# ShreenathKR2000/DFU-Multimodal

Measured on AMD Instinct MI355X. Metric: images/sec (fusion fwd+bwd, bs=64/GPU), higher is better.
Workload: dtype fwd ResNet50 bf16x3, ViT-B/16 Blocks fp16 (fp32 accumulate, residual stream, statistics); bwd bf16 MFMA; fp32 master weights / AdamW

## Files before the change

### dfu-multimodal_amd/csrc/bn.hip

```cpp
#include "common.h"

namespace {

constexpr int FIN_WAVES = 16;

DFU_DEV void st_sc1_f64(double* p, double v) {
  __hip_atomic_store((unsigned long long*)p, (unsigned long long)__double_as_longlong(v),
                     __ATOMIC_RELAXED, __HIP_MEMORY_SCOPE_AGENT);
}
DFU_DEV double ld_sc1_f64(const double* p) {
  return __longlong_as_double((long long)__hip_atomic_load((unsigned long long*)p, __ATOMIC_RELAXED,
                                                          __HIP_MEMORY_SCOPE_AGENT));
}

DFU_DEV bool last_slice(int* counter, int S, int* flag) {
  asm volatile("s_waitcnt vmcnt(0)" ::: "memory");
  __syncthreads();
  if (threadIdx.x == 0) {
    const int old = __hip_atomic_fetch_add(counter, 1, __ATOMIC_RELAXED, __HIP_MEMORY_SCOPE_AGENT);
    const int last = old == S - 1;
    if (last) __hip_atomic_store(counter, 0, __ATOMIC_RELAXED, __HIP_MEMORY_SCOPE_AGENT);
    *flag = last;
  }
  __syncthreads();
// ... 295 lines not shown
    }
  };
  if (FIXED) load_coef((threadIdx.x & (cv - 1)) * 8);
  for (int64_t i = blockIdx.x * (int64_t)blockDim.x + threadIdx.x; i < n;
       i += (int64_t)gridDim.x * blockDim.x) {
    if (!FIXED) load_coef((int)(i % cv) * 8);
    float g[8], yy[8], oo[8];
    const u32x4 gv = *(const u32x4*)(dout + i * 8), yv = *(const u32x4*)(y + i * 8);
    u32x4 ov = {};
    if constexpr (RELU == 1) ov = *(const u32x4*)(out + i * 8);
    if constexpr (RELU == 3) ov[0] = ((const uint8_t*)out)[i];
    unpack8(gv, g);
    unpack8(yv, yy);
    unpack8(ov, oo);
    relu_mask8<RELU>(oo, yy, sc, sf, g, ov[0]);
    if (dres) *(u32x4*)(dres + i * 8) = pack8(g);
    float d[8];
#pragma unroll
    for (int e = 0; e < 8; ++e) d[e] = fmaf(ka[e], g[e], fmaf(kb[e], yy[e], kc[e]));
    *(u32x4*)(dy + i * 8) = pack8(d);
  }
}

__global__ __launch_bounds__(256) void k_bn_tile_stats(const bf16_t* __restrict__ x, int M, int C,
                                                       float* __restrict__ stats) {
  __shared__ float red[4][64];
  const int lane = threadIdx.x & 63, g = threadIdx.x >> 6;
  const int c = blockIdx.y * 64 + lane;
  const int r0 = blockIdx.x * 128, nb = min(128, M - r0);
  const int ra = r0 + g * 32, rb = min(r0 + nb, ra + 32);
  float v[32];
#pragma unroll
  for (int i = 0; i < 32; ++i) {
    const int r = ra + i;
    v[i] = (c < C && r < rb) ? bf2f(x[(int64_t)r * C + c]) : 0.f;
  }
  float s = 0.f;
#pragma unroll
  for (int i = 0; i < 32; ++i) s += v[i];
  red[g][lane] = s;
  __syncthreads();
  const float tot = red[0][lane] + red[1][lane] + red[2][lane] + red[3][lane];
  const float mu = tot / (float)nb;
  __syncthreads();
  float q = 0.f;
#pragma unroll
// ... 169 lines not shown
                          stream);
}

extern "C" int dfu_bn_bwd_apply(const void* dout, const void* y, const void* out, int32_t relu,
                                const float* scale, const float* shift, const float* mean,
                                const float* invstd, const float* coef, int64_t M, int32_t C,
                                void* dy, void* dres, void* stream) {
  DFU_CHECK_ARG(dout && y && mean && invstd && coef && dy && C % 8 == 0 && M > 0 && relu >= 0 &&
                    relu <= 3,
                "dfu_bn_bwd_apply: bad args");
  DFU_CHECK_ARG((relu != 1 && relu != 3) || out, "dfu_bn_bwd_apply: relu=1/3 needs out/mask");
  DFU_CHECK_ARG(relu != 2 || (scale && shift), "dfu_bn_bwd_apply: relu=2 needs scale/shift");
  const bool fx = fixed_channels(C);
  auto kern = relu == 1   ? (fx ? k_bn_bwd_apply<1, true> : k_bn_bwd_apply<1, false>)
              : relu == 2 ? (fx ? k_bn_bwd_apply<2, true> : k_bn_bwd_apply<2, false>)
              : relu == 3 ? (fx ? k_bn_bwd_apply<3, true> : k_bn_bwd_apply<3, false>)
                          : (fx ? k_bn_bwd_apply<0, true> : k_bn_bwd_apply<0, false>);
  hipLaunchKernelGGL(kern, dim3(grid_for(M * C / 8)), dim3(256), 0, (hipStream_t)stream,
                     (const bf16_t*)dout, (const bf16_t*)y, (const bf16_t*)out, scale, shift, mean,
                     invstd, coef, M, C, (bf16_t*)dy, (bf16_t*)dres);
  DFU_LAUNCH_CHECK();
  return DFU_OK;
}
```

### dfu-multimodal_amd/csrc/precise.hip

```cpp
#include "common.h"

namespace {

constexpr int TPB = 256;

inline unsigned nblocks(int64_t n, int per_block = TPB) {
  int64_t b = (n + per_block - 1) / per_block;
  if (b > 65535 * 4) b = 65535 * 4;
  return (unsigned)(b < 1 ? 1 : b);
}

DFU_DEV void split8(const float* f, float* hi, float* lo) {
#pragma unroll
  for (int e = 0; e < 8; ++e) {
    hi[e] = bf2f(f2bf(f[e]));
    lo[e] = f[e] - hi[e];
  }
}

DFU_DEV void st_triple8(bf16_t* row, int C, int c, const float* f, int pattern) {
  float hi[8], lo[8];
  split8(f, hi, lo);
  const u32x4 h = pack8(hi), l = pack8(lo);
  *(u32x4*)(row + c) = h;
// ... 67 lines not shown
    } else {
      bf16_t* o = out + t * 3 * C + c;
      o[0] = h;
      o[C] = h;
      o[2 * C] = l;
    }
  }
}

DFU_DEV void st_pair8(bf16_t* hi, bf16_t* lo, int64_t e, const float* f) {
  float h[8], l[8];
  split8(f, h, l);
  *(u32x4*)(hi + e) = pack8(h);
  *(u32x4*)(lo + e) = pack8(l);
}
DFU_DEV void ld8_pair(const bf16_t* hi, const bf16_t* lo, int64_t e, float* f) {
  float h[8], l[8];
  unpack8(*(const u32x4*)(hi + e), h);
  unpack8(*(const u32x4*)(lo + e), l);
#pragma unroll
  for (int i = 0; i < 8; ++i) f[i] = h[i] + l[i];
}

__global__ void k_bn_apply_x3(const void* __restrict__ y, const bf16_t* __restrict__ y_lo,
                              const float* __restrict__ scale,
                              const float* __restrict__ shift, const void* __restrict__ res,
                              const bf16_t* __restrict__ res_lo, int res_mode, int relu,
                              bf16_t* __restrict__ out_lo, bf16_t* __restrict__ out_bf,
                              float* __restrict__ out_f32, bf16_t* __restrict__ y_bf,
                              uint8_t* __restrict__ relu_mask, int64_t M, int C, int cv_log2) {
  const int cv = C / 8;
  const int64_t n = M * cv;
  for (int64_t i = blockIdx.x * (int64_t)blockDim.x + threadIdx.x; i < n;
       i += (int64_t)gridDim.x * blockDim.x) {
    const int64_t m = i >> cv_log2;
    const int c = (int)(i & (cv - 1)) * 8;
    const int64_t e = m * C + c;
    float f[8], r[8], sc[8], sh[8];
    {
      const f32x4 s0 = *(const f32x4*)(scale + c), s1 = *(const f32x4*)(scale + c + 4);
      const f32x4 h0 = *(const f32x4*)(shift + c), h1 = *(const f32x4*)(shift + c + 4);
#pragma unroll
      for (int k = 0; k < 4; ++k) {
        sc[k] = s0[k];
        sc[k + 4] = s1[k];
        sh[k] = h0[k];
        sh[k + 4] = h1[k];
      }
    }
    if (y_lo) {
      ld8_pair((const bf16_t*)y, y_lo, e, f);
    } else {
      ld8_f32((const float*)y + e, f);
      if (y_bf) *(u32x4*)(y_bf + e) = pack8(f);
    }
    if (res_mode == 1) ld8_f32((const float*)res + e, r);
    else if (res_mode == 2) ld8_pair((const bf16_t*)res, res_lo, e, r);
#pragma unroll
    for (int k = 0; k < 8; ++k) {
      float v = fmaf(f[k], sc[k], sh[k]);
      if (res_mode) v += r[k];
      f[k] = relu ? fmaxf(v, 0.f) : v;
    }
    if (out_lo) st_pair8(out_bf, out_lo, e, f);
    else if (out_bf) *(u32x4*)(out_bf + e) = pack8(f);
    if (out_f32) st8_f32(out_f32 + e, f);
    if (relu_mask) {
      unsigned bits = 0;
#pragma unroll
      for (int k = 0; k < 8; ++k) bits |= (unsigned)(f[k] > 0.f) << k;
      relu_mask[i] = (uint8_t)bits;
    }
  }
}

__global__ void k_maxpool_fwd_x3(const float* __restrict__ x, int B, int H, int W, int C,
                                 bf16_t* __restrict__ y_lo, bf16_t* __restrict__ y_bf,
                                 uint8_t* __restrict__ am, int P, int Q) {
  const int cv = C / 8;
  const int64_t n = (int64_t)B * P * Q * cv;
// ... 203 lines not shown
                    (pattern != 2 || seg % 32 == 0) &&
                    (!hi_out || (ld_hi % 8 == 0 && ld_hi >= seg)),
                "dfu_split_x3: bad args (seg %% 8 == 0, seg >= cols, pattern 0/1/2; 2: seg %% 32 == 0)");
  const int64_t n = (int64_t)rows * (seg / 8);
  if (n == 0) return DFU_OK;
  hipLaunchKernelGGL(k_split_x3, dim3(nblocks(n)), dim3(TPB), 0, (hipStream_t)stream, in, ld_in,
                     rows, cols, seg, (bf16_t*)out, pattern, (bf16_t*)hi_out, ld_hi);
  DFU_LAUNCH_CHECK();
  return DFU_OK;
}

extern "C" int dfu_pack_conv_weight_x3(const float* w, void* out, int32_t K, int32_t C, int32_t R,
                                       int32_t S, int32_t pattern, void* stream) {
  DFU_CHECK_ARG(w && out && K > 0 && C > 0 && R > 0 && S > 0 &&
                    (pattern == 1 || (pattern == 2 && C % 32 == 0)),
                "dfu_pack_conv_weight_x3: bad args (pattern 1, or 2 with C %% 32 == 0)");
  const int64_t n = (int64_t)K * R * S * C;
  hipLaunchKernelGGL(k_pack_conv_weight_x3, dim3(nblocks(n)), dim3(TPB), 0, (hipStream_t)stream,
                     w, (bf16_t*)out, K, C, R, S, pattern);
  DFU_LAUNCH_CHECK();
  return DFU_OK;
}

extern "C" int dfu_bn_apply_x3(const void* y, const void* y_lo, const float* scale,
                               const float* shift, const void* residual,
                               const void* residual_lo, int32_t res_mode,
                               int32_t relu, void* out_lo, void* out_bf16, float* out_f32,
                               void* y_bf16, uint8_t* relu_mask, int64_t M, int32_t C,
                               void* stream) {
  const int cv = C / 8;
  int cv_log2 = 0;
  while ((1 << cv_log2) < cv) ++cv_log2;
  DFU_CHECK_ARG(C % 8 == 0 && cv > 0 && (1 << cv_log2) == cv,
                "dfu_bn_apply_x3: C / 8 must be a power of two (C=%d)", C);
  DFU_CHECK_ARG((((uintptr_t)scale | (uintptr_t)shift) & 15) == 0,
                "dfu_bn_apply_x3: scale/shift must be 16-byte aligned");
  DFU_CHECK_ARG(y && scale && shift && C % 8 == 0 && M >= 0 && res_mode >= 0 && res_mode <= 2 &&
                    (res_mode == 0 || residual) && (res_mode != 2 || residual_lo) &&
                    (!out_lo || out_bf16),
                "dfu_bn_apply_x3: bad args");
  const int64_t n = M * (C / 8);
  if (n == 0) return DFU_OK;
  hipLaunchKernelGGL(k_bn_apply_x3, dim3(nblocks(n)), dim3(TPB), 0, (hipStream_t)stream, y,
                     (const bf16_t*)y_lo, scale, shift, residual, (const bf16_t*)residual_lo,
                     res_mode, relu, (bf16_t*)out_lo,
                     (bf16_t*)out_bf16, out_f32, (bf16_t*)y_bf16, relu_mask, M, C, cv_log2);
  DFU_LAUNCH_CHECK();
  return DFU_OK;
}

extern "C" int dfu_maxpool_fwd_x3(const float* x, int32_t B, int32_t H, int32_t W, int32_t C,
                                  void* y_lo, void* y_bf16, uint8_t* argmax, int32_t P, int32_t Q,
                                  void* stream) {
  DFU_CHECK_ARG(x && y_lo && y_bf16 && argmax && C % 8 == 0, "dfu_maxpool_fwd_x3: bad args");
  DFU_CHECK_ARG(P == (H - 1) / 2 + 1 && Q == (W - 1) / 2 + 1, "dfu_maxpool_fwd_x3: bad P/Q");
  const int64_t n = (int64_t)B * P * Q * (C / 8);
  hipLaunchKernelGGL(k_maxpool_fwd_x3, dim3(nblocks(n)), dim3(TPB), 0, (hipStream_t)stream, x, B,
                     H, W, C, (bf16_t*)y_lo, (bf16_t*)y_bf16, argmax, P, Q);
  DFU_LAUNCH_CHECK();
  return DFU_OK;
}

extern "C" int dfu_maxpool_bn_fwd_x3(const void* y, const void* y_lo, const float* scale,
                                     const float* shift, int32_t B, int32_t H, int32_t W,
                                     int32_t C, void* out_lo, void* out_bf16, uint8_t* argmax,
                                     uint8_t* relu_mask, int32_t P, int32_t Q, void* stream) {
  const int cv = C / 8;
  int cv_log2 = 0;
  while ((1 << cv_log2) < cv) ++cv_log2;
  DFU_CHECK_ARG(y && y_lo && scale && shift && out_lo && out_bf16 && argmax && C % 8 == 0 &&
                    cv > 0 && (1 << cv_log2) == cv && P == (H - 1) / 2 + 1 &&
// ... 65 lines not shown
```

### dfu-multimodal_amd/dfu_hip/functional.py

```python
import math
import os
import weakref

import torch

from . import _lib as L
from . import ops
from .streams import (current_stream, join_grad_streams, new_stream, on_stream,
                      side_stream, stream_wait, wgrad_stream)
from .grads import (arm_backward_join, disarm_backward_join, grad_buffer,
                    grad_or_none, grads_done, register_backward_end_hook,
                    register_grad_ready_hook, remove_backward_end_hook, remove_grad_ready_hook,
                    wants)
from .optim import x3_pair_weight

BF16 = torch.bfloat16
F32 = torch.float32

PRECISIONS = ("bf16", "bf16x3", "mixed", "parity")
STAGE_MODES = ("bf16", "bf16x3", "fp16")
DEFAULT_PRECISION = "parity"
_precision = [DEFAULT_PRECISION]


# ... 208 lines not shown
                w._dfu_shadow_x3_version = w._version
            return sh
    if _X3_PAIRS:
        if w.shape[2] == 1 and w.shape[3] == 1:
            return ops.split_x3(w.detach().reshape(w.shape[0], -1), ops.X3_PAIRS)
        return ops.pack_conv_weight_x3(w.detach(), ops.X3_PAIRS)
    if w.shape[2] == 1 and w.shape[3] == 1:
        return weight_x3_rows(w)
    return ops.pack_conv_weight_x3(w.detach())


def _take_x3(x):
    hi = rows_view(nhwc_bf16(x.detach()))
    lo = getattr(x, "_dfu_lo", None)
    if lo is not None:
        try:
            del x._dfu_lo
        except AttributeError:
            pass
        return hi, lo
    return hi, torch.zeros_like(hi)


class BNState:

    def __init__(self, bn, M, C, device):
        self.bn = bn
        self.M, self.C = M, C
        self.training = bn.training or not bn.track_running_stats
        self.coef4 = _empty((4, C), F32, device)
        self.scale, self.shift, self.mean, self.invstd = self.coef4.unbind(0)

    def forward_coeffs(self, stats):
        bn = self.bn
        if self.training:
            track = bn.track_running_stats and bn.training
            mom = bn.momentum if bn.momentum is not None else 0.1
            mp = module_param
            ops.bn_finalize(stats, self.M, self.C, mp(bn, "weight"), mp(bn, "bias"), bn.eps, mom,
                            mp(bn, "running_mean") if track else None,
                            mp(bn, "running_var") if track else None,
                            mp(bn, "num_batches_tracked") if track else None,
                            self.mean, self.invstd, self.scale, self.shift)
        else:
            ops.bn_eval_coeffs(bn.weight, bn.bias, bn.running_mean, bn.running_var, bn.eps,
                               self.scale, self.shift)
            self.mean.copy_(bn.running_mean)
            ops.bn_eval_coeffs(None, None, bn.running_mean, bn.running_var, bn.eps,
                               self.invstd, _empty((self.C,), F32, self.mean.device))

    def backward(self, dout, y, out, relu, dy, dres):
        bn = self.bn
        w, b = module_param(bn, "weight"), module_param(bn, "bias")
        dgamma = grad_or_none(w)
        dbeta = grad_or_none(b)
        ops.bn_bwd(dout, y, out, relu, self.mean, self.invstd, w, self.M, self.C, dy,
                   dres, dgamma, dbeta, batch_stats=self.training, scale=self.scale,
                   shift=self.shift)
        grads_done(w, b)


def gemm_wgrad(N, K, rows, dy, x, dw, ld_dy=None, ld_x=None):
    ops.gemm(N, K, rows, dy, N if ld_dy is None else ld_dy, x,
             x.stride(0) if ld_x is None else ld_x, dw, K, a_mode=L.OPND_MNMAJOR,
             b_mode=L.OPND_MNMAJOR, epilogue=L.EPI_F32_ACC)


def gemm_dgrad_f32(rows, N, K, dy, w):
    dx = _empty((rows, N), F32, dy.device)
    ops.gemm(rows, N, K, dy, K, w, N, dx, N, b_mode=L.OPND_MNMAJOR, epilogue=L.EPI_F32)
    return dx


def conv_fwd(x_rows, geom, w_krsc, y, stats):
    g = geom
    M = g.n * g.p * g.q
    if g.plain:
        ops.gemm(M, g.k, g.c, x_rows, g.c, w_krsc, g.c, y, g.k, epilogue=L.EPI_BF16_STATS,
                 stats=stats)
    else:
        K = g.r * g.s * g.c
        ops.gemm(M, g.k, K, x_rows, 0, w_krsc, K, y, g.k, a_mode=L.OPND_CONV_FWD,
# ... 171 lines not shown
        dx = im2col_conv_dx(dy, wb, g) if ctx.x_requires_grad else None
        return dx, None, None, None, None


def _fire_grad_hooks(probe, grad):
    for hook in list((probe._backward_hooks or {}).values()):
        hook(grad)


def conv_bn(xrows, geom, w, bnmod, relu, residual=None, mask=None):
    dev = xrows.device
    M = geom.n * geom.p * geom.q
    y = _empty((M, geom.k), BF16, dev)
    stats = _empty((ops.stats_tiles(M), 2, geom.k), F32, dev)
    conv_fwd(xrows, geom, w, y, stats)
    st = BNState(bnmod, M, geom.k, dev)
    st.forward_coeffs(stats)
    out = _empty((M, geom.k), BF16, dev)
    ops.bn_apply(y, st.scale, st.shift, residual, relu, out, M, geom.k, mask=mask)
    return y, out, st


def conv_bn_x3(xpair, geom, w3x, bnmod, relu, res=None, res_mode=0, want_pair=True,
               want_f32=False):
    dev = xpair[0].device
    M = geom.n * geom.p * geom.q
    y = _empty((M, geom.k), BF16, dev)
    y_lo = _empty((M, geom.k), BF16, dev)
    stats = _empty((ops.stats_tiles(M), 2, geom.k), F32, dev)
    conv_fwd_x3(xpair, geom, w3x, y, stats, y_lo=y_lo)
    st = BNState(bnmod, M, geom.k, dev)
    st.forward_coeffs(stats)
    out = _empty((M, geom.k), BF16, dev) if want_pair else None
    lo = _empty((M, geom.k), BF16, dev) if want_pair else None
    of = _empty((M, geom.k), F32, dev) if want_f32 else None
    rhi, rlo = res if res_mode == 2 else (res, None)
    mask = _empty((M * geom.k // 8,), torch.uint8, dev) if relu else None
    ops.bn_apply_x3(y, st.scale, st.shift, rhi, res_mode, relu, M, geom.k, out_lo=lo,
                    out_bf16=out, out_f32=of, residual_lo=rlo, y_lo=y_lo, relu_mask=mask)
    return y, out, lo, of, st, mask


class BottleneckFn(torch.autograd.Function):

    @staticmethod
    def forward(ctx, x, *params_and_mod):
        mod = params_and_mod[-1]
        mm = mod._modules
        x3mode = _x3(mod)
        xin3 = _take_x3(x) if x3mode else None
        x = nhwc_bf16(x.detach())
        B, Cin, H, W = x.shape
        xr = rows_view(x)
        g1 = _geom(mm["conv1"], B, H, W)
        g2 = _geom(mm["conv2"], B, g1.p, g1.q)
        g3 = _geom(mm["conv3"], B, g2.p, g2.q)
        down = mm.get("downsample")
        geo = (g1, g2, g3, _geom(down[0], B, H, W) if down is not None else None)
        w1 = conv_weight_bf16(mm["conv1"].weight)
        w2 = conv_weight_bf16(mm["conv2"].weight)
# ... 21 lines not shown
        y1, a1, s1 = conv_bn(xr, g1, w1, mm["bn1"], True)
        y2, a2, s2 = conv_bn(a1, g2, w2, mm["bn2"], True)
        wd, yd, sd, idn = None, None, None, xr
        if gd is not None:
            dconv, dbn = mm["downsample"][0], mm["downsample"][1]
            wd = conv_weight_bf16(dconv.weight)
            yd, idn, sd = conv_bn(xr, gd, wd, dbn, False)
        mask3 = _empty((y2.shape[0] * g3.k // 8,), torch.uint8, xr.device)
        y3, out, s3 = conv_bn(a2, g3, w3, mm["bn3"], True, residual=idn, mask=mask3)
        return (y1, y2, y3, yd), (a1, a2), (s1, s2, s3, sd), (None, None, mask3), wd, out, None

    @staticmethod
    def _forward_x3(mm, xin3, geo):
        g1, g2, g3, gd = geo
        y1, a1, a1_lo, _, s1, m1 = conv_bn_x3(xin3, g1, conv_weight_x3(mm["conv1"].weight),
                                               mm["bn1"], True)
        y2, a2, a2_lo, _, s2, m2 = conv_bn_x3((a1, a1_lo), g2,
                                               conv_weight_x3(mm["conv2"].weight), mm["bn2"], True)
        del a1_lo
        wd, yd, sd, res, res_mode = None, None, None, xin3, 2
        if gd is not None:
            dconv, dbn = mm["downsample"][0], mm["downsample"][1]
            wd = conv_weight_bf16(dconv.weight)
            yd, _, _, res, sd, _ = conv_bn_x3(xin3, gd, conv_weight_x3(dconv.weight), dbn, False,
                                              want_pair=False, want_f32=True)
            res_mode = 1
        y3, out, out_lo, _, s3, mask3 = conv_bn_x3((a2, a2_lo), g3,
                                                    conv_weight_x3(mm["conv3"].weight), mm["bn3"],
                                                    True, res=res, res_mode=res_mode)
        return (y1, y2, y3, yd), (a1, a2), (s1, s2, s3, sd), (m1, m2, mask3), wd, out, out_lo

    @staticmethod
    def backward(ctx, gout):
        xr, y1, a1, y2, a2, y3, mask3, w1, w2, w3, yd, wd = ctx.saved_tensors
        mm = ctx.mod._modules
        g1, g2, g3, gd = ctx.geo
        s1, s2, s3, sd = ctx.bns
        B, Cin, H, W = ctx.shape
        g = rows_view(nhwc_bf16(gout))
        dy3 = torch.empty_like(y3)
        dres = torch.empty_like(y3)
        s3.backward(g, y3, mask3, 3, dy3, dres)
        dyd = None
        if yd is not None:
            dyd = torch.empty_like(yd)
            sd.backward(dres, yd, None, False, dyd, None)
            conv_param_wgrad(mm.get("downsample")[0], dyd, xr, gd)
        da2 = torch.empty_like(a2)
        conv_dgrad(dy3, g3, w3, da2, w_t=conv1x1_weight_T(mm["conv3"], g3))
        if ctx.probes is not None:
            _fire_grad_hooks(ctx.probes[1], from_rows(da2, B, g2.p, g2.q, g2.k))
        conv_param_wgrad(mm["conv3"], dy3, a2, g3)
        dy2 = torch.empty_like(y2)
        m1, m2 = ctx.masks
        s2.backward(da2, y2, m2, 3 if ctx.x3 else 2, dy2, None)
        da1 = torch.empty_like(a1)
        conv_dgrad(dy2, g2, w2, da1, w_flip=None if g2.stride != 1 else
                   conv_weight_flipped(mm["conv2"].weight))
        if ctx.probes is not None:
            _fire_grad_hooks(ctx.probes[0], from_rows(da1, B, g1.p, g1.q, g1.k))
        conv_param_wgrad(mm["conv2"], dy2, a1, g2)
        dy1 = torch.empty_like(y1)
        s1.backward(da1, y1, m1, 3 if ctx.x3 else 2, dy1, None)
        dx = None
        if ctx.x_requires_grad:
            dxr = _empty((y1.shape[0], Cin), BF16, xr.device)
            w1t = conv1x1_weight_T(mm["conv1"], g1)
            if dyd is None:
                conv_dgrad(dy1, g1, w1, dxr, add=dres, w_t=w1t)
# ... 537 lines not shown
```

### dfu-multimodal_amd/dfu_hip/ops.py

```python
import ctypes

import numpy as np
import torch

from . import _lib as L
from ._lib import check
from .streams import (TILE_COUNTERS, current_stream, on_stream, refuse_in_capture,
                      stream_ptr, stream_wait, tile_counters)

BF16 = torch.bfloat16
F32 = torch.float32
F16 = torch.float16


def lib():
    return L.load()


def ptr(t):
    return None if t is None else t.data_ptr()


def _req(t, dtype, name):
    if t.dtype != dtype:
# ... 347 lines not shown
_BN_BWD_WS = {}


def bn_bwd(dout, y, out, relu, mean, invstd, gamma, M, C, dy, dres, dgamma, dbeta,
           batch_stats=True, scale=None, shift=None):
    relu = int(relu)
    if relu == 2 and (scale is None or shift is None):
        raise ValueError("bn_bwd: relu=2 needs the forward scale/shift")
    lb = lib()
    nb = _BN_BWD_WS.get((M, C))
    if nb is None:
        nb = _BN_BWD_WS[(M, C)] = int(lb.dfu_bn_bwd_ws_bytes(M, C))
    dev = y.device
    ws = torch.empty((nb + 7) // 8, dtype=torch.float64, device=dev)
    cnt = tile_counters(dev)
    rc = lb.dfu_bn_bwd(ptr(dout), y.data_ptr(), ptr(out), relu, ptr(scale), ptr(shift),
                       mean.data_ptr(), invstd.data_ptr(), ptr(gamma), M, C, int(batch_stats),
                       ptr(dgamma), ptr(dbeta), dy.data_ptr(), ptr(dres), ws.data_ptr(), nb,
                       cnt.data_ptr(), cnt.numel(), stream_ptr())
    if rc:
        check(rc, "dfu_bn_bwd")


def maxpool_fwd(x, B, H, W, C, scale=None, shift=None):
    P = (H - 1) // 2 + 1
    Q = (W - 1) // 2 + 1
    y = torch.empty((B, P, Q, C), dtype=BF16, device=x.device)
    am = torch.empty((B, P, Q, C), dtype=torch.uint8, device=x.device)
    if scale is None:
        check(lib().dfu_maxpool_fwd(ptr(x), B, H, W, C, ptr(y), ptr(am), P, Q, stream_ptr()),
              "dfu_maxpool_fwd")
    else:
        check(lib().dfu_maxpool_bn_fwd(ptr(x), ptr(scale), ptr(shift), B, H, W, C, ptr(y),
                                       ptr(am), P, Q, stream_ptr()), "dfu_maxpool_bn_fwd")
    return y, am, P, Q


def maxpool_bwd(dy, am, B, H, W, C, P, Q):
    dx = torch.empty((B, H, W, C), dtype=BF16, device=dy.device)
    check(lib().dfu_maxpool_bwd(ptr(dy), ptr(am), B, H, W, C, P, Q, ptr(dx), stream_ptr()),
          "dfu_maxpool_bwd")
    return dx


def avgpool_fwd(x, B, HW, C):
    y = torch.empty((B, C), dtype=F32, device=x.device)
# ... 290 lines not shown
    sn, sc, sh, sw = x.stride()
    check(lib().dfu_im2col_f32_x3(ptr(x), sn, sc, sh, sw, B, C, H, W, R, S, stride, pad, P, Q,
                                  ptr(hi), ptr(lo), Kp, stream_ptr()), "dfu_im2col_f32_x3")
    return (hi, lo), P, Q


def patchify_f32_x3(x, ps):
    _req(x, F32, "patchify_f32_x3")
    B, C, H, W = x.shape
    out = torch.empty((B * (H // ps) * (W // ps), 3 * C * ps * ps), dtype=BF16, device=x.device)
    sn, sc, sh, sw = x.stride()
    check(lib().dfu_patchify_f32_x3(ptr(x), sn, sc, sh, sw, B, C, H, W, ps, ptr(out),
                                    stream_ptr()), "dfu_patchify_f32_x3")
    return out


def bn_apply_x3(y, scale, shift, residual, res_mode, relu, M, C, out_lo=None, out_bf16=None,
                out_f32=None, y_bf16=None, residual_lo=None, y_lo=None, relu_mask=None):
    _req(y, F32 if y_lo is None else BF16, "bn_apply_x3")
    check(lib().dfu_bn_apply_x3(ptr(y), ptr(y_lo), ptr(scale), ptr(shift), ptr(residual),
                                ptr(residual_lo), int(res_mode), int(relu), ptr(out_lo),
                                ptr(out_bf16), ptr(out_f32), ptr(y_bf16), ptr(relu_mask), int(M),
                                int(C), stream_ptr()), "dfu_bn_apply_x3")


def maxpool_fwd_x3(x, B, H, W, C):
    _req(x, F32, "maxpool_fwd_x3")
    P = (H - 1) // 2 + 1
    Q = (W - 1) // 2 + 1
    lo = torch.empty((B * P * Q, C), dtype=BF16, device=x.device)
    y = torch.empty((B, P, Q, C), dtype=BF16, device=x.device)
    am = torch.empty((B, P, Q, C), dtype=torch.uint8, device=x.device)
    check(lib().dfu_maxpool_fwd_x3(ptr(x), B, H, W, C, ptr(lo), ptr(y), ptr(am), P, Q,
                                   stream_ptr()), "dfu_maxpool_fwd_x3")
    return lo, y, am, P, Q


def stem_conv_x3(x, w, stride=2, pad=3, want_col=True):
    _req(x, F32, "stem_conv_x3")
    _req(w, F32, "stem_conv_x3")
    B, C, H, W = x.shape
    K, Cw, R, S = w.shape
    P = (H + 2 * pad - R) // stride + 1
    Q = (W + 2 * pad - S) // stride + 1
    M = B * P * Q
    y = torch.empty((M, K), dtype=BF16, device=x.device)
# ... 269 lines not shown
```

### include/dfu_hip.h

```cpp
#ifndef DFU_HIP_H
#define DFU_HIP_H
#include <stdint.h>

#ifdef __cplusplus
extern "C" {
#endif

#define DFU_OK 0
#define DFU_E_INVALID 1001
#define DFU_E_UNSUPPORTED 1002

const char* dfu_last_error_string(void);
int dfu_version(void);
int dfu_zero(void* ptr, int64_t bytes, void* stream);

int dfu_stream_create(int32_t priority, void** stream);
int dfu_stream_destroy(void* stream);
int dfu_stream_wait(void* waiter, void* producer);
int dfu_stream_capture_status(void* stream, int32_t* status);
int dfu_streams_abort_capture(void* const* streams, int32_t n, int32_t* still_capturing);

enum dfu_operand_mode {
  DFU_OPND_KMAJOR = 0,
  DFU_OPND_MNMAJOR = 1,
// ... 119 lines not shown
                 int32_t relu, void* out, int64_t M, int32_t C, void* stream);
int dfu_bn_apply_mask(const void* y, const float* scale, const float* shift,
                      const void* residual, int32_t relu, void* out, uint8_t* mask, int64_t M,
                      int32_t C, void* stream);
int dfu_bn_bwd_blocks(int64_t M, int32_t C);
int dfu_bn_bwd_reduce(const void* dout, const void* y, const void* out, int32_t relu,
                      const float* scale, const float* shift, const float* mean,
                      const float* invstd, int64_t M, int32_t C, float* partial, void* stream);
int dfu_bn_bwd_finalize(const float* partial, int32_t blocks, int64_t M, int32_t C,
                        const float* gamma, const float* invstd, int32_t batch_stats,
                        float* dgamma, float* dbeta, float* coef, double* ws, int32_t* counters,
                        int32_t ncounters, void* stream);
int64_t dfu_bn_bwd_finalize_ws_bytes(int32_t blocks, int32_t C);
int dfu_bn_bwd_apply(const void* dout, const void* y, const void* out, int32_t relu,
                     const float* scale, const float* shift, const float* mean,
                     const float* invstd, const float* coef, int64_t M, int32_t C, void* dy,
                     void* dres, void* stream);
int64_t dfu_bn_bwd_ws_bytes(int64_t M, int32_t C);
int dfu_bn_bwd(const void* dout, const void* y, const void* out, int32_t relu, const float* scale,
               const float* shift, const float* mean, const float* invstd, const float* gamma,
               int64_t M, int32_t C, int32_t batch_stats, float* dgamma, float* dbeta, void* dy,
               void* dres, void* ws, int64_t ws_bytes, int32_t* counters, int32_t ncounters,
               void* stream);

int dfu_maxpool_fwd(const void* x, int32_t B, int32_t H, int32_t W, int32_t C, void* y,
                    uint8_t* argmax, int32_t P, int32_t Q, void* stream);
int dfu_maxpool_bn_fwd(const void* x, const float* scale, const float* shift, int32_t B,
                       int32_t H, int32_t W, int32_t C, void* y, uint8_t* argmax, int32_t P,
                       int32_t Q, void* stream);
int dfu_maxpool_bwd(const void* dy, const uint8_t* argmax, int32_t B, int32_t H, int32_t W,
                    int32_t C, int32_t P, int32_t Q, void* dx, void* stream);
int dfu_avgpool_fwd(const void* x, int32_t B, int32_t HW, int32_t C, float* y, void* stream);
int dfu_avgpool_bwd(const float* dy, int32_t B, int32_t HW, int32_t C, void* dx, void* stream);

int dfu_layernorm_fwd(const float* x, int64_t ldx, int32_t rows, int32_t D, const float* gamma,
                      const float* beta, float eps, void* out, int64_t ldo, int32_t out_bf16,
                      float* mean, float* rstd, void* stream);
int dfu_ln_bwd_blocks(int32_t rows);
int dfu_layernorm_bwd(const void* dy, int64_t lddy, int32_t dy_bf16, const float* x,
                      int64_t ldx, const float* mean, const float* rstd, const float* gamma,
                      int32_t rows, int32_t D, float* gx, int64_t ldg, void* gx_bf16,
                      float* partial, float* gsum_partial, void* stream);
int dfu_reduce_partials(const float* partial, int32_t blocks, int32_t nvec, int32_t D,
                        float* out0, float* out1, void* stream);
#define DFU_REDUCE_BATCH 8
typedef struct dfu_reduce_entry {
// ... 55 lines not shown
                   int64_t x3_begin, int64_t x3_end, void* stream);
int dfu_step_increment(int64_t* step_dev, void* stream);
int dfu_argmax_rows(const float* x, int32_t rows, int32_t C, int64_t* out, void* stream);
int dfu_softmax_rows(const float* x, int32_t rows, int32_t C, float* out, void* stream);
int dfu_metrics_accumulate(const float* logits, const int64_t* labels, int32_t rows, int32_t C,
                           const float* loss, int64_t* confusion, double* loss_sum,
                           int64_t* batches, void* stream);

enum dfu_x3_pattern { DFU_X3_A = 0, DFU_X3_B = 1, DFU_X3_PAIRS = 2 };
int dfu_split_x3(const float* in, int64_t ld_in, int32_t rows, int32_t cols, int32_t seg,
                 void* out, int32_t pattern, void* hi_out, int64_t ld_hi, void* stream);
int dfu_pack_conv_weight_x3(const float* w, void* out, int32_t K, int32_t C, int32_t R, int32_t S,
                            int32_t pattern, void* stream);
int dfu_im2col_f32_x3(const float* x, int64_t sn, int64_t sc, int64_t sh, int64_t sw, int32_t B,
                      int32_t C, int32_t H, int32_t W, int32_t R, int32_t S, int32_t stride,
                      int32_t pad, int32_t P, int32_t Q, void* out, void* out_lo, int32_t Kp,
                      void* stream);
int dfu_patchify_f32_x3(const float* x, int64_t sn, int64_t sc, int64_t sh, int64_t sw, int32_t B,
                        int32_t C, int32_t H, int32_t W, int32_t ps, void* out, void* stream);
int dfu_bn_apply_x3(const void* y, const void* y_lo, const float* scale, const float* shift,
                    const void* residual, const void* residual_lo, int32_t res_mode, int32_t relu,
                    void* out_lo, void* out_bf16, float* out_f32, void* y_bf16,
                    uint8_t* relu_mask, int64_t M, int32_t C, void* stream);
int dfu_maxpool_fwd_x3(const float* x, int32_t B, int32_t H, int32_t W, int32_t C, void* y_lo,
                       void* y_bf16, uint8_t* argmax, int32_t P, int32_t Q, void* stream);
int dfu_stem_conv_x3(const float* x, int64_t sn, int64_t sc, int64_t sh, int64_t sw, int32_t B,
                     int32_t C, int32_t H, int32_t W, const float* w, int32_t K, int32_t R,
                     int32_t S, int32_t stride, int32_t pad, void* y, void* y_lo, float* stats,
                     void* col, void* stream);
int64_t dfu_stem_wgrad_ws_bytes(int32_t B, int32_t H, int32_t W);
int dfu_stem_wgrad_x3(const float* x, int64_t sn, int64_t sc, int64_t sh, int64_t sw, int32_t B,
                      int32_t C, int32_t H, int32_t W, const void* dy, int32_t K, int32_t R,
                      int32_t S, int32_t stride, int32_t pad, float* dw, float* slab,
                      int64_t slab_bytes, void* stream);
int dfu_maxpool_bn_fwd_x3(const void* y, const void* y_lo, const float* scale, const float* shift,
                          int32_t B, int32_t H, int32_t W, int32_t C, void* out_lo,
                          void* out_bf16, uint8_t* argmax, uint8_t* relu_mask, int32_t P,
                          int32_t Q, void* stream);
int dfu_avgpool_fwd_x3(const void* hi, const void* lo, int32_t B, int32_t HW, int32_t C, float* y,
                       void* stream);
int dfu_layernorm_fwd_x3(const float* x, int64_t ldx, int32_t rows, int32_t D,
                         const float* gamma, const float* beta, float eps, void* out3,
                         void* out_bf16, float* mean, float* rstd, void* stream);
int dfu_layernorm_fwd_h16(const float* x, int64_t ldx, int32_t rows, int32_t D,
                          const float* gamma, const float* beta, float eps, void* out_f16,
                          void* out_bf16, float* mean, float* rstd, void* stream);
// ... 65 lines not shown
```

Measured before the change: 3118.

## Fuse downsample BN into bottleneck residual apply and pair BN backward

In the forward pass, the downsample branch's BN apply (which wrote an fp32 residual) is folded into the main bn3 apply kernel through a new res_mode that normalises the downsample conv output inline. In the backward pass, a paired kernel computes both BN reductions and both dgrad applies from one read of dout, the mask and both y tensors, so the dres intermediate is no longer written and read back. This cuts kernel launches and memory traffic in each ResNet downsample block. In exchange the paired reduce keeps three per-thread accumulator sets and a larger shared-memory array, and the path is gated by an environment flag.

```diff
diff --git a/dfu-multimodal_amd/csrc/bn.hip b/dfu-multimodal_amd/csrc/bn.hip
--- a/dfu-multimodal_amd/csrc/bn.hip
+++ b/dfu-multimodal_amd/csrc/bn.hip
@@ -341,6 +341,139 @@
   }
 }
 
+__global__ void k_bn_bwd_reduce_pair(const bf16_t* __restrict__ dout,
+                                     const uint8_t* __restrict__ mask,
+                                     const bf16_t* __restrict__ ya, const bf16_t* __restrict__ yb,
+                                     const float* __restrict__ mean_a,
+                                     const float* __restrict__ invstd_a,
+                                     const float* __restrict__ mean_b,
+                                     const float* __restrict__ invstd_b, int64_t M, int C,
+                                     int rows_per_block, float* __restrict__ partial_a,
+                                     float* __restrict__ partial_b) {
+  __shared__ float red[3][256][8];
+  const int cv = C / 8;
+  const int ct_n = min(cv, 64);
+  const int rl_n = 256 / ct_n;
+  const int ct = threadIdx.x % ct_n, rl = threadIdx.x / ct_n;
+  const int c8 = blockIdx.x * ct_n + ct;
+  const int c0 = c8 * 8;
+  const int64_t r0 = (int64_t)blockIdx.y * rows_per_block;
+  const int64_t r1 = min(M, r0 + rows_per_block);
+  float sg[8] = {0, 0, 0, 0, 0, 0, 0, 0}, sgxa[8] = {0, 0, 0, 0, 0, 0, 0, 0};
+  float sgxb[8] = {0, 0, 0, 0, 0, 0, 0, 0};
+  float mua[8], isa[8], mub[8], isb[8];
+#pragma unroll
+  for (int e = 0; e < 8; ++e) {
+    mua[e] = mean_a[c0 + e]; isa[e] = invstd_a[c0 + e];
+    mub[e] = mean_b[c0 + e]; isb[e] = invstd_b[c0 + e];
+  }
+  for (int64_t rb = r0 + rl; rb < r1; rb += (int64_t)rl_n * RED_U) {
+    u32x4 gv[RED_U], av[RED_U], bv[RED_U];
+    unsigned mb[RED_U];
+#pragma unroll
+    for (int u = 0; u < RED_U; ++u) {
+      const int64_t r = rb + (int64_t)u * rl_n;
+      const int64_t o = (r < r1 ? r : r0) * C + c0;
+      gv[u] = *(const u32x4*)(dout + o);
+      av[u] = *(const u32x4*)(ya + o);
+      bv[u] = *(const u32x4*)(yb + o);
+      mb[u] = mask[o / 8];
+    }
+#pragma unroll
+    for (int u = 0; u < RED_U; ++u) {
+      if (rb + (int64_t)u * rl_n >= r1) continue;
+      float g[8], a[8], b[8];
+      unpack8(gv[u], g);
+      unpack8(av[u], a);
+      unpack8(bv[u], b);
+      relu_mask8<3>(nullptr, nullptr, nullptr, nullptr, g, mb[u]);
+#pragma unroll
+      for (int e = 0; e < 8; ++e) {
+        sg[e] += g[e];
+        sgxa[e] += g[e] * (a[e] - mua[e]) * isa[e];
+        sgxb[e] += g[e] * (b[e] - mub[e]) * isb[e];
+      }
+    }
+  }
+#pragma unroll
+  for (int e = 0; e < 8; ++e) {
+    red[0][threadIdx.x][e] = sg[e];
+    red[1][threadIdx.x][e] = sgxa[e];
+    red[2][threadIdx.x][e] = sgxb[e];
+  }
+  __syncthreads();
+  if (rl == 0) {
+    for (int l = 1; l < rl_n; ++l) {
+#pragma unroll
+      for (int e = 0; e < 8; ++e) {
+        sg[e] += red[0][l * ct_n + ct][e];
+        sgxa[e] += red[1][l * ct_n + ct][e];
+        sgxb[e] += red[2][l * ct_n + ct][e];
+      }
+    }
+    const int64_t p0 = ((int64_t)blockIdx.y * 2 + 0) * C + c0;
+    const int64_t p1 = ((int64_t)blockIdx.y * 2 + 1) * C + c0;
+#pragma unroll
+    for (int e = 0; e < 8; ++e) {
+      partial_a[p0 + e] = sg[e]; partial_a[p1 + e] = sgxa[e];
+      partial_b[p0 + e] = sg[e]; partial_b[p1 + e] = sgxb[e];
+    }
+  }
+}
+
+template <bool FIXED>
+__global__ void k_bn_bwd_apply_pair(const bf16_t* __restrict__ dout,
+                                    const uint8_t* __restrict__ mask,
+                                    const bf16_t* __restrict__ ya, const bf16_t* __restrict__ yb,
+                                    const float* __restrict__ mean_a,
+                                    const float* __restrict__ invstd_a,
+                                    const float* __restrict__ coef_a,
+                                    const float* __restrict__ mean_b,
+                                    const float* __restrict__ invstd_b,
+                                    const float* __restrict__ coef_b, int64_t M, int C,
+                                    bf16_t* __restrict__ dya, bf16_t* __restrict__ dyb) {
+  const int cv = C / 8;
+  const int64_t n = M * cv;
+  float aa[8], ab[8], ac[8], ba[8], bb[8], bc[8];
+  auto load3 = [&](const float* coef, const float* mean, const float* invstd, int c0, float* ka,
+                   float* kb, float* kc) {
+#pragma unroll
+    for (int e = 0; e < 8; ++e) {
+      const int c = c0 + e;
+      const float k = coef[3 * c], m1 = coef[3 * c + 1], m2 = coef[3 * c + 2];
+      const float is = invstd[c];
+      ka[e] = k;
+      kb[e] = -k * m2 * is;
+      kc[e] = k * (m2 * is * mean[c] - m1);
+    }
+  };
+  auto load_coef = [&](int c0) {
+    load3(coef_a, mean_a, invstd_a, c0, aa, ab, ac);
+    load3(coef_b, mean_b, invstd_b, c0, ba, bb, bc);
+  };
+  if (FIXED) load_coef((threadIdx.x & (cv - 1)) * 8);
+  for (int64_t i = blockIdx.x * (int64_t)blockDim.x + threadIdx.x; i < n;
+       i += (int64_t)gridDim.x * blockDim.x) {
+    if (!FIXED) load_coef((int)(i % cv) * 8);
+    const u32x4 gv = *(const u32x4*)(dout + i * 8);
+    const u32x4 av = *(const u32x4*)(ya + i * 8), bv = *(const u32x4*)(yb + i * 8);
+    const unsigned mb = mask[i];
+    float g[8], a[8], b[8];
+    unpack8(gv, g);
+    unpack8(av, a);
+    unpack8(bv, b);
+    relu_mask8<3>(nullptr, nullptr, nullptr, nullptr, g, mb);
+    float da[8], db[8];
+#pragma unroll
+    for (int e = 0; e < 8; ++e) {
+      da[e] = fmaf(aa[e], g[e], fmaf(ab[e], a[e], ac[e]));
+      db[e] = fmaf(ba[e], g[e], fmaf(bb[e], b[e], bc[e]));
+    }
+    *(u32x4*)(dya + i * 8) = pack8(da);
+    *(u32x4*)(dyb + i * 8) = pack8(db);
+  }
+}
+
 __global__ __launch_bounds__(256) void k_bn_tile_stats(const bf16_t* __restrict__ x, int M, int C,
                                                        float* __restrict__ stats) {
   __shared__ float red[4][64];
@@ -556,3 +689,55 @@
   DFU_LAUNCH_CHECK();
   return DFU_OK;
 }
+
+extern "C" int64_t dfu_bn_bwd_pair_ws_bytes(int64_t M, int32_t C) {
+  return 2 * dfu_bn_bwd_ws_bytes(M, C);
+}
+
+extern "C" int dfu_bn_bwd_pair(const void* dout, const uint8_t* mask, const void* y_a,
+                               const float* mean_a, const float* invstd_a, const float* gamma_a,
+                               const void* y_b, const float* mean_b, const float* invstd_b,
+                               const float* gamma_b, int64_t M, int32_t C, int32_t batch_stats,
+                               float* dgamma_a, float* dbeta_a, float* dgamma_b, float* dbeta_b,
+                               void* dy_a, void* dy_b, void* ws, int64_t ws_bytes,
+                               int32_t* counters, int32_t ncounters, void* stream) {
+  DFU_CHECK_ARG(dout && mask && y_a && mean_a && invstd_a && y_b && mean_b && invstd_b && dy_a &&
+                    dy_b && C > 0 && C % 8 == 0 && M > 0,
+                "dfu_bn_bwd_pair: bad args");
+  const int cv = C / 8;
+  const int ct_n = cv < 64 ? cv : 64;
+  DFU_CHECK_ARG(256 % ct_n == 0 && cv % ct_n == 0, "dfu_bn_bwd_pair: C=%d unsupported", C);
+  DFU_CHECK_ARG(ws && ws_bytes >= dfu_bn_bwd_pair_ws_bytes(M, C) && ((uintptr_t)ws & 15) == 0,
+                "dfu_bn_bwd_pair: workspace of dfu_bn_bwd_pair_ws_bytes(M, C) bytes (16-B "
+                "aligned) needed");
+  const int rpb = bwd_rows_per_block(M, C);
+  const int blocks = dfu_bn_bwd_blocks(M, C);
+  const int64_t fin = dfu_bn_bwd_finalize_ws_bytes(blocks, C);
+  double* fws_a = fin > 0 ? (double*)ws : nullptr;
+  double* fws_b = fin > 0 ? (double*)((char*)ws + fin) : nullptr;
+  float* partial_a = (float*)((char*)ws + 2 * fin);
+  float* partial_b = partial_a + (int64_t)blocks * 2 * C;
+  float* coef_a = partial_b + (int64_t)blocks * 2 * C;
+  float* coef_b = coef_a + 3LL * C;
+  hipLaunchKernelGGL(k_bn_bwd_reduce_pair, dim3(cv / ct_n, blocks), dim3(256), 0,
+                     (hipStream_t)stream, (const bf16_t*)dout, mask, (const bf16_t*)y_a,
+                     (const bf16_t*)y_b, mean_a, invstd_a, mean_b, invstd_b, M, C, rpb, partial_a,
+                     partial_b);
+  DFU_LAUNCH_CHECK();
+  int rc = dfu_bn_bwd_finalize(partial_a, blocks, M, C, gamma_a, invstd_a, batch_stats, dgamma_a,
+                               dbeta_a, coef_a, fws_a, fws_a ? counters : nullptr,
+                               fws_a ? ncounters : 0, stream);
+  if (rc != DFU_OK) return rc;
+  rc = dfu_bn_bwd_finalize(partial_b, blocks, M, C, gamma_b, invstd_b, batch_stats, dgamma_b,
+                           dbeta_b, coef_b, fws_b, fws_b ? counters : nullptr,
+                           fws_b ? ncounters : 0, stream);
+  if (rc != DFU_OK) return rc;
+  const bool fx = fixed_channels(C);
+  hipLaunchKernelGGL(fx ? k_bn_bwd_apply_pair<true> : k_bn_bwd_apply_pair<false>,
+                     dim3(grid_for(M * C / 8)), dim3(256), 0, (hipStream_t)stream,
+                     (const bf16_t*)dout, mask, (const bf16_t*)y_a, (const bf16_t*)y_b, mean_a,
+                     invstd_a, coef_a, mean_b, invstd_b, coef_b, M, C, (bf16_t*)dy_a,
+                     (bf16_t*)dy_b);
+  DFU_LAUNCH_CHECK();
+  return DFU_OK;
+}
diff --git a/dfu-multimodal_amd/csrc/precise.hip b/dfu-multimodal_amd/csrc/precise.hip
--- a/dfu-multimodal_amd/csrc/precise.hip
+++ b/dfu-multimodal_amd/csrc/precise.hip
@@ -113,10 +113,25 @@
   for (int i = 0; i < 8; ++i) f[i] = h[i] + l[i];
 }
 
+DFU_DEV void ld_coef8(const float* __restrict__ scale, const float* __restrict__ shift, int c,
+                      float* sc, float* sh) {
+  const f32x4 s0 = *(const f32x4*)(scale + c), s1 = *(const f32x4*)(scale + c + 4);
+  const f32x4 h0 = *(const f32x4*)(shift + c), h1 = *(const f32x4*)(shift + c + 4);
+#pragma unroll
+  for (int k = 0; k < 4; ++k) {
+    sc[k] = s0[k];
+    sc[k + 4] = s1[k];
+    sh[k] = h0[k];
+    sh[k + 4] = h1[k];
+  }
+}
+
 __global__ void k_bn_apply_x3(const void* __restrict__ y, const bf16_t* __restrict__ y_lo,
                               const float* __restrict__ scale,
                               const float* __restrict__ shift, const void* __restrict__ res,
-                              const bf16_t* __restrict__ res_lo, int res_mode, int relu,
+                              const bf16_t* __restrict__ res_lo,
+                              const float* __restrict__ scale_d,
+                              const float* __restrict__ shift_d, int res_mode, int relu,
                               bf16_t* __restrict__ out_lo, bf16_t* __restrict__ out_bf,
                               float* __restrict__ out_f32, bf16_t* __restrict__ y_bf,
                               uint8_t* __restrict__ relu_mask, int64_t M, int C, int cv_log2) {
@@ -127,18 +142,9 @@
     const int64_t m = i >> cv_log2;
     const int c = (int)(i & (cv - 1)) * 8;
     const int64_t e = m * C + c;
-    float f[8], r[8], sc[8], sh[8];
-    {
-      const f32x4 s0 = *(const f32x4*)(scale + c), s1 = *(const f32x4*)(scale + c + 4);
-      const f32x4 h0 = *(const f32x4*)(shift + c), h1 = *(const f32x4*)(shift + c + 4);
-#pragma unroll
-      for (int k = 0; k < 4; ++k) {
-        sc[k] = s0[k];
-        sc[k + 4] = s1[k];
-        sh[k] = h0[k];
-        sh[k + 4] = h1[k];
-      }
-    }
+    float f[8], r[8], sc[8], sh[8], scd[8] = {}, shd[8] = {};
+    ld_coef8(scale, shift, c, sc, sh);
+    if (res_mode == 3) ld_coef8(scale_d, shift_d, c, scd, shd);
     if (y_lo) {
       ld8_pair((const bf16_t*)y, y_lo, e, f);
     } else {
@@ -146,7 +152,11 @@
       if (y_bf) *(u32x4*)(y_bf + e) = pack8(f);
     }
     if (res_mode == 1) ld8_f32((const float*)res + e, r);
-    else if (res_mode == 2) ld8_pair((const bf16_t*)res, res_lo, e, r);
+    else if (res_mode >= 2) ld8_pair((const bf16_t*)res, res_lo, e, r);
+    if (res_mode == 3) {
+#pragma unroll
+      for (int k = 0; k < 8; ++k) r[k] = fmaf(r[k], scd[k], shd[k]);
+    }
 #pragma unroll
     for (int k = 0; k < 8; ++k) {
       float v = fmaf(f[k], sc[k], sh[k]);
@@ -396,31 +406,56 @@
   return DFU_OK;
 }
 
+namespace {
+int bn_apply_x3_launch(const char* who, const void* y, const void* y_lo, const float* scale,
+                       const float* shift, const void* residual, const void* residual_lo,
+                       const float* scale_d, const float* shift_d, int res_mode, int relu,
+                       void* out_lo, void* out_bf16, float* out_f32, void* y_bf16,
+                       uint8_t* relu_mask, int64_t M, int C, void* stream) {
+  const int cv = C / 8;
+  int cv_log2 = 0;
+  while ((1 << cv_log2) < cv) ++cv_log2;
+  DFU_CHECK_ARG(C % 8 == 0 && cv > 0 && (1 << cv_log2) == cv,
+                "%s: C / 8 must be a power of two (C=%d)", who, C);
+  DFU_CHECK_ARG((((uintptr_t)scale | (uintptr_t)shift | (uintptr_t)scale_d |
+                  (uintptr_t)shift_d) & 15) == 0,
+                "%s: scale/shift must be 16-byte aligned", who);
+  DFU_CHECK_ARG(y && scale && shift && M >= 0 && res_mode >= 0 && res_mode <= 3 &&
+                    (res_mode == 0 || residual) && (res_mode < 2 || residual_lo) &&
+                    (res_mode != 3 || (scale_d && shift_d)) && (!out_lo || out_bf16),
+                "%s: bad args", who);
+  const int64_t n = M * cv;
+  if (n == 0) return DFU_OK;
+  hipLaunchKernelGGL(k_bn_apply_x3, dim3(nblocks(n)), dim3(TPB), 0, (hipStream_t)stream, y,
+                     (const bf16_t*)y_lo, scale, shift, residual, (const bf16_t*)residual_lo,
+                     scale_d, shift_d, res_mode, relu, (bf16_t*)out_lo, (bf16_t*)out_bf16,
+                     out_f32, (bf16_t*)y_bf16, relu_mask, M, C, cv_log2);
+  DFU_LAUNCH_CHECK();
+  return DFU_OK;
+}
+}
+
 extern "C" int dfu_bn_apply_x3(const void* y, const void* y_lo, const float* scale,
                                const float* shift, const void* residual,
                                const void* residual_lo, int32_t res_mode,
                                int32_t relu, void* out_lo, void* out_bf16, float* out_f32,
                                void* y_bf16, uint8_t* relu_mask, int64_t M, int32_t C,
                                void* stream) {
-  const int cv = C / 8;
-  int cv_log2 = 0;
-  while ((1 << cv_log2) < cv) ++cv_log2;
-  DFU_CHECK_ARG(C % 8 == 0 && cv > 0 && (1 << cv_log2) == cv,
-                "dfu_bn_apply_x3: C / 8 must be a power of two (C=%d)", C);
-  DFU_CHECK_ARG((((uintptr_t)scale | (uintptr_t)shift) & 15) == 0,
-                "dfu_bn_apply_x3: scale/shift must be 16-byte aligned");
-  DFU_CHECK_ARG(y && scale && shift && C % 8 == 0 && M >= 0 && res_mode >= 0 && res_mode <= 2 &&
-                    (res_mode == 0 || residual) && (res_mode != 2 || residual_lo) &&
-                    (!out_lo || out_bf16),
-                "dfu_bn_apply_x3: bad args");
-  const int64_t n = M * (C / 8);
-  if (n == 0) return DFU_OK;
-  hipLaunchKernelGGL(k_bn_apply_x3, dim3(nblocks(n)), dim3(TPB), 0, (hipStream_t)stream, y,
-                     (const bf16_t*)y_lo, scale, shift, residual, (const bf16_t*)residual_lo,
-                     res_mode, relu, (bf16_t*)out_lo,
-                     (bf16_t*)out_bf16, out_f32, (bf16_t*)y_bf16, relu_mask, M, C, cv_log2);
-  DFU_LAUNCH_CHECK();
-  return DFU_OK;
+  DFU_CHECK_ARG(res_mode >= 0 && res_mode <= 2, "dfu_bn_apply_x3: bad args (res_mode=%d)",
+                res_mode);
+  return bn_apply_x3_launch("dfu_bn_apply_x3", y, y_lo, scale, shift, residual, residual_lo,
+                            nullptr, nullptr, res_mode, relu, out_lo, out_bf16, out_f32, y_bf16,
+                            relu_mask, M, C, stream);
+}
+
+extern "C" int dfu_bn_apply_x3_ds(const void* y, const void* y_lo, const float* scale,
+                                  const float* shift, const void* yd, const void* yd_lo,
+                                  const float* scale_d, const float* shift_d, int32_t relu,
+                                  void* out_lo, void* out_bf16, float* out_f32, void* y_bf16,
+                                  uint8_t* relu_mask, int64_t M, int32_t C, void* stream) {
+  return bn_apply_x3_launch("dfu_bn_apply_x3_ds", y, y_lo, scale, shift, yd, yd_lo, scale_d,
+                            shift_d, 3, relu, out_lo, out_bf16, out_f32, y_bf16, relu_mask, M, C,
+                            stream);
 }
 
 extern "C" int dfu_maxpool_fwd_x3(const float* x, int32_t B, int32_t H, int32_t W, int32_t C,
diff --git a/dfu-multimodal_amd/dfu_hip/functional.py b/dfu-multimodal_amd/dfu_hip/functional.py
--- a/dfu-multimodal_amd/dfu_hip/functional.py
+++ b/dfu-multimodal_amd/dfu_hip/functional.py
@@ -254,6 +254,9 @@
     return hi, torch.zeros_like(hi)
 
 
+_BN_PAIR = os.environ.get("DFU_BN_PAIR", "1") != "0"
+
+
 class BNState:
 
     def __init__(self, bn, M, C, device):
@@ -290,6 +293,16 @@
                    dres, dgamma, dbeta, batch_stats=self.training, scale=self.scale,
                    shift=self.shift)
         grads_done(w, b)
+
+    def backward_pair(self, other, dout, mask, y, y_other, dy, dy_other):
+        sides, params = [], []
+        for st, yy in ((self, y), (other, y_other)):
+            w, b = module_param(st.bn, "weight"), module_param(st.bn, "bias")
+            sides.append((yy, st.mean, st.invstd, w, grad_or_none(w), grad_or_none(b)))
+            params += [w, b]
+        ops.bn_bwd_pair(dout, mask, sides[0], sides[1], self.M, self.C, dy, dy_other,
+                        batch_stats=self.training)
+        grads_done(*params)
 
 
 def gemm_wgrad(N, K, rows, dy, x, dw, ld_dy=None, ld_x=None):
@@ -507,7 +520,7 @@
 
 
 def conv_bn_x3(xpair, geom, w3x, bnmod, relu, res=None, res_mode=0, want_pair=True,
-               want_f32=False):
+               want_f32=False, apply=True):
     dev = xpair[0].device
     M = geom.n * geom.p * geom.q
     y = _empty((M, geom.k), BF16, dev)
@@ -516,11 +529,18 @@
     conv_fwd_x3(xpair, geom, w3x, y, stats, y_lo=y_lo)
     st = BNState(bnmod, M, geom.k, dev)
     st.forward_coeffs(stats)
+    if not apply:
+        return y, y_lo, st
     out = _empty((M, geom.k), BF16, dev) if want_pair else None
     lo = _empty((M, geom.k), BF16, dev) if want_pair else None
     of = _empty((M, geom.k), F32, dev) if want_f32 else None
+    mask = _empty((M * geom.k // 8,), torch.uint8, dev) if relu else None
+    if res_mode == 3:
+        yd, yd_lo, sd = res
+        ops.bn_apply_x3_ds(y, y_lo, st.scale, st.shift, yd, yd_lo, sd.scale, sd.shift, relu, M,
+                           geom.k, out_lo=lo, out_bf16=out, out_f32=of, relu_mask=mask)
+        return y, out, lo, of, st, mask
     rhi, rlo = res if res_mode == 2 else (res, None)
-    mask = _empty((M * geom.k // 8,), torch.uint8, dev) if relu else None
     ops.bn_apply_x3(y, st.scale, st.shift, rhi, res_mode, relu, M, geom.k, out_lo=lo,
                     out_bf16=out, out_f32=of, residual_lo=rlo, y_lo=y_lo, relu_mask=mask)
     return y, out, lo, of, st, mask
@@ -588,9 +608,14 @@
         if gd is not None:
             dconv, dbn = mm["downsample"][0], mm["downsample"][1]
             wd = conv_weight_bf16(dconv.weight)
-            yd, _, _, res, sd, _ = conv_bn_x3(xin3, gd, conv_weight_x3(dconv.weight), dbn, False,
-                                              want_pair=False, want_f32=True)
-            res_mode = 1
+            if _BN_PAIR:
+                yd, yd_lo, sd = conv_bn_x3(xin3, gd, conv_weight_x3(dconv.weight), dbn, False,
+                                           apply=False)
+                res, res_mode = (yd, yd_lo, sd), 3
+            else:
+                yd, _, _, res, sd, _ = conv_bn_x3(xin3, gd, conv_weight_x3(dconv.weight), dbn,
+                                                  False, want_pair=False, want_f32=True)
+                res_mode = 1
         y3, out, out_lo, _, s3, mask3 = conv_bn_x3((a2, a2_lo), g3,
                                                     conv_weight_x3(mm["conv3"].weight), mm["bn3"],
                                                     True, res=res, res_mode=res_mode)
@@ -605,12 +630,17 @@
         B, Cin, H, W = ctx.shape
         g = rows_view(nhwc_bf16(gout))
         dy3 = torch.empty_like(y3)
-        dres = torch.empty_like(y3)
-        s3.backward(g, y3, mask3, 3, dy3, dres)
-        dyd = None
+        dyd, dres = None, None
+        if yd is not None and _BN_PAIR and s3.training == sd.training:
+            dyd = torch.empty_like(yd)
+            s3.backward_pair(sd, g, mask3, y3, yd, dy3, dyd)
+        else:
+            dres = torch.empty_like(y3)
+            s3.backward(g, y3, mask3, 3, dy3, dres)
+            if yd is not None:
+                dyd = torch.empty_like(yd)
+                sd.backward(dres, yd, None, False, dyd, None)
         if yd is not None:
-            dyd = torch.empty_like(yd)
-            sd.backward(dres, yd, None, False, dyd, None)
             conv_param_wgrad(mm.get("downsample")[0], dyd, xr, gd)
         da2 = torch.empty_like(a2)
         conv_dgrad(dy3, g3, w3, da2, w_t=conv1x1_weight_T(mm["conv3"], g3))
diff --git a/dfu-multimodal_amd/dfu_hip/ops.py b/dfu-multimodal_amd/dfu_hip/ops.py
--- a/dfu-multimodal_amd/dfu_hip/ops.py
+++ b/dfu-multimodal_amd/dfu_hip/ops.py
@@ -393,6 +393,31 @@
         check(rc, "dfu_bn_bwd")
 
 
+_BN_BWD_PAIR_WS = {}
+
+
+def bn_bwd_pair(dout, mask, a, b, M, C, dy_a, dy_b, batch_stats=True):
+    ya, mean_a, invstd_a, gamma_a, dgamma_a, dbeta_a = a
+    yb, mean_b, invstd_b, gamma_b, dgamma_b, dbeta_b = b
+    _req(dout, BF16, "bn_bwd_pair")
+    _req(ya, BF16, "bn_bwd_pair")
+    _req(yb, BF16, "bn_bwd_pair")
+    lb = lib()
+    nb = _BN_BWD_PAIR_WS.get((M, C))
+    if nb is None:
+        nb = _BN_BWD_PAIR_WS[(M, C)] = int(lb.dfu_bn_bwd_pair_ws_bytes(M, C))
+    dev = ya.device
+    ws = torch.empty((nb + 7) // 8, dtype=torch.float64, device=dev)
+    cnt = tile_counters(dev)
+    rc = lb.dfu_bn_bwd_pair(ptr(dout), ptr(mask), ptr(ya), ptr(mean_a), ptr(invstd_a),
+                            ptr(gamma_a), ptr(yb), ptr(mean_b), ptr(invstd_b), ptr(gamma_b), M, C,
+                            int(batch_stats), ptr(dgamma_a), ptr(dbeta_a), ptr(dgamma_b),
+                            ptr(dbeta_b), ptr(dy_a), ptr(dy_b), ws.data_ptr(), nb,
+                            cnt.data_ptr(), cnt.numel(), stream_ptr())
+    if rc:
+        check(rc, "dfu_bn_bwd_pair")
+
+
 def maxpool_fwd(x, B, H, W, C, scale=None, shift=None):
     P = (H - 1) // 2 + 1
     Q = (W - 1) // 2 + 1
@@ -729,6 +754,17 @@
                                 ptr(residual_lo), int(res_mode), int(relu), ptr(out_lo),
                                 ptr(out_bf16), ptr(out_f32), ptr(y_bf16), ptr(relu_mask), int(M),
                                 int(C), stream_ptr()), "dfu_bn_apply_x3")
+
+
+def bn_apply_x3_ds(y, y_lo, scale, shift, yd, yd_lo, scale_d, shift_d, relu, M, C, out_lo=None,
+                   out_bf16=None, out_f32=None, relu_mask=None):
+    for t in (y, y_lo, yd, yd_lo):
+        _req(t, BF16, "bn_apply_x3_ds")
+    check(lib().dfu_bn_apply_x3_ds(ptr(y), ptr(y_lo), ptr(scale), ptr(shift), ptr(yd),
+                                   ptr(yd_lo), ptr(scale_d), ptr(shift_d), int(relu),
+                                   ptr(out_lo), ptr(out_bf16), ptr(out_f32), None,
+                                   ptr(relu_mask), int(M), int(C), stream_ptr()),
+          "dfu_bn_apply_x3_ds")
 
 
 def maxpool_fwd_x3(x, B, H, W, C):
diff --git a/include/dfu_hip.h b/include/dfu_hip.h
--- a/include/dfu_hip.h
+++ b/include/dfu_hip.h
@@ -165,6 +165,13 @@
                int64_t M, int32_t C, int32_t batch_stats, float* dgamma, float* dbeta, void* dy,
                void* dres, void* ws, int64_t ws_bytes, int32_t* counters, int32_t ncounters,
                void* stream);
+int64_t dfu_bn_bwd_pair_ws_bytes(int64_t M, int32_t C);
+int dfu_bn_bwd_pair(const void* dout, const uint8_t* mask, const void* y_a, const float* mean_a,
+                    const float* invstd_a, const float* gamma_a, const void* y_b,
+                    const float* mean_b, const float* invstd_b, const float* gamma_b, int64_t M,
+                    int32_t C, int32_t batch_stats, float* dgamma_a, float* dbeta_a,
+                    float* dgamma_b, float* dbeta_b, void* dy_a, void* dy_b, void* ws,
+                    int64_t ws_bytes, int32_t* counters, int32_t ncounters, void* stream);
 
 int dfu_maxpool_fwd(const void* x, int32_t B, int32_t H, int32_t W, int32_t C, void* y,
                     uint8_t* argmax, int32_t P, int32_t Q, void* stream);
@@ -266,6 +273,11 @@
                     const void* residual, const void* residual_lo, int32_t res_mode, int32_t relu,
                     void* out_lo, void* out_bf16, float* out_f32, void* y_bf16,
                     uint8_t* relu_mask, int64_t M, int32_t C, void* stream);
+int dfu_bn_apply_x3_ds(const void* y, const void* y_lo, const float* scale, const float* shift,
+                       const void* yd, const void* yd_lo, const float* scale_d,
+                       const float* shift_d, int32_t relu, void* out_lo, void* out_bf16,
+                       float* out_f32, void* y_bf16, uint8_t* relu_mask, int64_t M, int32_t C,
+                       void* stream);
 int dfu_maxpool_fwd_x3(const float* x, int32_t B, int32_t H, int32_t W, int32_t C, void* y_lo,
                        void* y_bf16, uint8_t* argmax, int32_t P, int32_t Q, void* stream);
 int dfu_stem_conv_x3(const float* x, int64_t sn, int64_t sc, int64_t sh, int64_t sw, int32_t B,
```

Result: no change. 3143, median of 6 (+0.8%).
